# xiezhy6/PASTA-GAN-plusplus

Hardware: AMD Instinct MI355X
Metric: 512-res try-on images/sec (SynthesisNetwork fwd) (higher is better)
Workload: dtype f32

## Files before the change

### include/pasta_gan_ops.h

```cpp
#ifndef PASTA_GAN_OPS_H
#define PASTA_GAN_OPS_H

#include <stdint.h>

#ifdef __cplusplus
extern "C" {
#endif

#define PG_ABI_VERSION 16

enum pg_dtype { PG_F32 = 0, PG_F16 = 1, PG_BF16 = 2, PG_F64 = 3 };

enum pg_error {
    PG_OK = 0,
    PG_ERR_INVALID_ARG = -1,
    PG_ERR_UNSUPPORTED = -2,
    PG_ERR_TOO_LARGE = -3
};

enum pg_act {
    PG_ACT_LINEAR = 1, PG_ACT_RELU = 2, PG_ACT_LRELU = 3, PG_ACT_TANH = 4, PG_ACT_SIGMOID = 5,
    PG_ACT_ELU = 6, PG_ACT_SELU = 7, PG_ACT_SOFTPLUS = 8, PG_ACT_SWISH = 9
};

int pg_bias_act(const void* x, const void* b, const void* xref, const void* yref, const void* dy, void* y,
                int dtype, int64_t sizeX, int sizeB, int64_t stepB,
                int grad, int act, float alpha, float gain, float clamp, void* stream);
int pg_bias_act_abi_version(void);

int64_t pg_bias_act_grad_bias_workspace(int dtype, int64_t sizeX, int sizeB, int64_t stepB);
int pg_bias_act_grad_bias(const void* dy, const void* yref, void* dx, void* db, void* workspace, int64_t workspace_bytes,
                          int dtype, int64_t sizeX, int sizeB, int64_t stepB,
                          int act, float alpha, float gain, float clamp, void* stream);

int pg_upfirdn2d(const void* x, const float* f, void* y, int dtype,
                 int N, int C, int inH, int inW, const int64_t xstride[4],
                 int fh, int fw, const int64_t fstride[2],
                 int outH, int outW, const int64_t ystride[4],
                 int upx, int upy, int downx, int downy, int padx0, int pady0,
                 int flip, float gain, void* stream);
int pg_upfirdn2d_with_odd_samples(const void* x, const float* f, void* y, float* y_odd, int dtype,
                                  int N, int C, int inH, int inW, const int64_t xstride[4],
// ... 86 lines not shown
    float*       s_norm[PG_MODCONV_PREP_MAX_JOBS];
    void*        s16[PG_MODCONV_PREP_MAX_JOBS];
    int          cout[PG_MODCONV_PREP_MAX_JOBS];
    int          cin[PG_MODCONV_PREP_MAX_JOBS];
    int          flags[PG_MODCONV_PREP_MAX_JOBS];
    int          njobs;
    int          half_dtype;
} pg_modconv_prep_jobs;
int pg_modconv_prep_batched(const pg_modconv_prep_jobs* jobs, int N, void* stream);

int pg_conv2d_up2_forward(const float* x, const float* packed, float* y, int N, int Cin, int H, int W, int Cout,
                          const int64_t ystride[4], const float* in_scale, const float* out_scale, void* stream);
int pg_conv2d_up2_splitk_plan(int N, int Cin, int H, int W, int Cout);
int pg_conv2d_up2_forward_splitk(const float* x, const float* packed, float* y, int N, int Cin, int H, int W, int Cout,
                                 const int64_t ystride[4], const float* in_scale, const float* out_scale, float* workspace, int ksplit, void* stream);

int64_t pg_conv2d_up2x3_packed_size(int Cout, int Cin);
int pg_conv2d_up2x3_pack_weight(const float* packed, void* packed_x3, int Cout, int Cin, void* stream);
int pg_conv2d_up2x3_forward(const float* x, const float* packed, const void* packed_x3, float* y, int N, int Cin, int H, int W, int Cout,
                            const int64_t ystride[4], const float* in_scale, const float* out_scale, float* edge_column, void* stream);

int64_t pg_conv2d_stem7x3_packed_size(int Cout);
int pg_conv2d_stem7x3_pack_weight(const float* w, void* packed, int Cout, float scale, int flip_hw, void* stream);
int pg_conv2d_stem7x3_forward(const float* x, const void* packed, float* y, int N, int H, int W, int Cout, const int64_t ystride[4],
                              const pg_conv2d_fusion* fusion, void* stream);

int pg_conv1x1_small(const float* x, const float* w, const float* styles, const float* bias, const float* skip, float* y,
                     int N, int Cin, int64_t HW, int Cout, float scale, float clamp, void* stream);

int pg_conv1x1_fold_prep(const float* wm, const float* bm, const float* wh, const float* bh, const float* styles, float* w_out, float* b_out,
                         int N, int Cm, int C, int Cout, void* stream);
int pg_conv1x1_fold_heads(const float* x, const float* x2, const float* w, const float* bias, const float* skip, float* y_a, float* y_b,
                          int N, int C1, int C2, int64_t HW, int Cout, int c_a, int n_skip, float clamp, void* stream);

int pg_conv3x3_cin1(const float* x, const float* w, float* y, int N, int H, int W, int Cout, float scale, int act, void* stream);

int pg_instance_norm_stats(const float* x, float* mean, float* rstd, int NC, int64_t HW, float eps, void* stream);
int pg_spade_norm(const float* x, const float* mean, const float* rstd, const float* gamma, const float* beta,
                  float* y, int NC, int64_t HW, void* stream);

#define PG_STATS16_MAX_CHUNKS 256
int pg_instance_norm_stats_cl16(const void* x, float* mean, float* rstd, float* workspace, int dtype, int N, int64_t HW, int C, float eps, void* stream);
int pg_spade_combine_cl16(const void* x, const float* mean, const float* rstd, const void* gamma_beta, void* y, int dtype, int N, int64_t HW, int C,
                          int act, float alpha, float gain, float clamp, void* stream);

int pg_spade_train_forward(const float* x, const float* mean, const float* rstd, const float* gamma, const float* beta, float* y,
                           int N, int C, int64_t HW, int64_t gamma_sample_stride, int64_t beta_sample_stride, void* stream);
int pg_spade_train_backward(const float* dy, const float* x, const float* mean, const float* rstd, const float* gamma, float* sums,
                            float* dx, float* dgamma, float* dbeta, int N, int C, int64_t HW,
                            int64_t gamma_sample_stride, int64_t dgamma_sample_stride, int64_t dbeta_sample_stride, void* stream);

int pg_spade_masked_sums(const float* feat, const float* mask, const float* denorm_mask, float* sums, float* counts,
                         int N, int C, int H, int W, void* stream);
int pg_spade_feat_assemble(const float* feat_upper, const float* feat_lower, const float* mask_upper, const float* mask_lower,
                           const float* denorm_mask_upper, const float* denorm_mask_lower,
                           const float* sums_upper, const float* sums_lower, const float* counts_upper, const float* counts_lower,
                           float* out, int N, int C, int H, int W, void* stream);
int pg_conv2d_abi_version(void);
int pg_conv2d_reserve_cus(int n);

int pg_conv2d_wgrad_plan(int N, int Cin, int OH, int OW, int Cout, int KH, int KW, int stride);
int pg_conv2d_wgrad(const float* x, const float* dy, float* dw, float* workspace,
                    int N, int Cin, int H, int W, int Cout, int KH, int KW, int stride, int pad_y, int pad_x, int OH, int OW,
                    int splits, void* stream);

int pg_conv2d16_wgrad_plan(int N, int Cin, int OH, int OW, int Cout, int KH, int KW, int stride);
// ... 213 lines not shown
```

### pasta-gan-plusplus_amd/torch_utils/custom_ops.py

```python

import concurrent.futures
import ctypes
import fcntl
import glob
import hashlib
import os
import re
import shutil
import subprocess
import sys

verbosity = 'brief'

CSRC_DIR = os.path.normpath(os.path.join(os.path.dirname(os.path.abspath(__file__)), '..', 'csrc'))
INCLUDE_DIR = os.path.normpath(os.path.join(CSRC_DIR, '..', '..', 'include'))
DEV_DIR = os.path.join(CSRC_DIR, 'dev')
OFFLOAD_ARCH = 'gfx950'
HIPCC_FLAGS = ['-O3', '-std=c++17', '-fPIC', '-fvisibility=hidden', f'--offload-arch={OFFLOAD_ARCH}']

PLUGIN_SOURCES = {
    'bias_act_plugin': ['bias_act.hip'],
    'upfirdn2d_plugin': ['upfirdn2d.hip'],
    'patch_routing_plugin': ['patch_routing.hip'],
    'augment_plugin': ['augment.hip'],
    'tryon_plugin': ['tryon.hip'],
    'tryon_front_plugin': ['tryon_front.hip'],
    'train_fetch_plugin': ['train_fetch.hip'],
    'snapshot_grid_plugin': ['snapshot_grid.hip'],
    'conv2d_plugin': ['conv2d.hip', 'conv2d_inst_k3s1.hip', 'conv2d_inst_k1s1.hip', 'conv2d_inst_k2x2.hip', 'conv2d_inst_k2x1.hip',
                      'conv2d_inst_k1x2.hip', 'conv2d_inst_k7s1.hip', 'conv2d_inst_k3s2.hip', 'conv2d_inst_k1s2.hip', 'conv2d_inst_wino.hip', 'conv2d_inst_wino4.hip', 'conv2d_inst_wino4s.hip', 'conv2d_inst_wino4t.hip', 'conv2d_inst_wino4x.hip', 'conv2d_inst_wino4xs.hip', 'conv2d_inst_wino4xt.hip', 'conv2d_inst_wino4b.hip', 'conv2d_inst_wino4bs.hip', 'conv2d_inst_up2.hip', 'conv2d_inst_stem7.hip', 'conv2d_inst_s1x1.hip',
                      'conv2d_wgrad.hip', 'conv2d16.hip', 'conv2d16_inst_k3s1.hip', 'conv2d16_inst_k3s1b.hip', 'conv2d16_inst_k1s1.hip', 'conv2d16_inst_k2x2.hip', 'conv2d16_inst_k2x1.hip',
                      'conv2d16_inst_k1x2.hip', 'conv2d16_inst_k3s2.hip', 'conv2d16_inst_up2f.hip', 'conv1x1_head16.hip', 'spade16.hip', 'conv1x1_fold.hip', 'optim.hip'],
}

ABI_VERSION = 16

_cached_plugins = dict()


class NativePlugin:

    def __init__(self, name, path, abi_name=None):
        self.name = name
        self.path = path
        self.lib = ctypes.CDLL(path)
        probe = getattr(self.lib, 'pg_' + (abi_name or name).replace('_plugin', '') + '_abi_version', None)
        if probe is None:
            raise RuntimeError(f'{path} does not export its ABI version; rebuild it from csrc/')
        probe.restype = ctypes.c_int
        if probe() != ABI_VERSION:
            raise RuntimeError(f'{path} implements ABI version {probe()}, the bindings expect {ABI_VERSION}; rebuild it from csrc/')

    def __repr__(self):
        return f'<NativePlugin {self.name} at {self.path}>'


def _find_hipcc():
    for cand in (os.environ.get('HIPCC'), shutil.which('hipcc'), '/opt/rocm/bin/hipcc'):
        if cand and os.path.isfile(cand):
            return cand
    return None


def _digest(sources, extra_flags):
    h = hashlib.md5()
    deps = sorted(set(list(sources) + glob.glob(os.path.join(CSRC_DIR, '*.h')) + glob.glob(os.path.join(INCLUDE_DIR, '*.h'))))
    for path in deps:
        h.update(os.path.basename(path).encode())
# ... 180 lines not shown
```

### pasta-gan-plusplus_amd/torch_utils/ops/conv2d_mfma.py

```python

import ctypes
import os

import torch

from .. import custom_ops
from . import _native as nat

ACT_INDEX = {'linear': 1, 'relu': 2, 'lrelu': 3, 'tanh': 4, 'sigmoid': 5, 'elu': 6, 'selu': 7, 'softplus': 8, 'swish': 9}

FUSED_ACTS = ('linear', 'relu', 'lrelu')

SUPPORTED = {(3, 3, 1), (1, 1, 1), (2, 2, 1), (2, 1, 1), (1, 2, 1), (7, 7, 1), (3, 3, 2), (1, 1, 2)}


class Fusion(ctypes.Structure):
    _fields_ = [
        ('in_scale', ctypes.c_void_p), ('in_bias', ctypes.c_void_p), ('in_act', ctypes.c_int), ('in_alpha', ctypes.c_float),
        ('in_gain', ctypes.c_float), ('in_clamp', ctypes.c_float),
        ('out_scale', ctypes.c_void_p), ('noise', ctypes.c_void_p), ('noise_batch_stride', ctypes.c_int64), ('noise_gain', ctypes.c_float),
        ('bias', ctypes.c_void_p), ('act', ctypes.c_int), ('alpha', ctypes.c_float), ('gain', ctypes.c_float), ('clamp', ctypes.c_float),
        ('residual', ctypes.c_void_p),
        ('spade_x', ctypes.c_void_p), ('spade_mean', ctypes.c_void_p), ('spade_rstd', ctypes.c_void_p),
        ('x2', ctypes.c_void_p), ('cin_split', ctypes.c_int),
# ... 90 lines not shown
        lib.pg_conv2d_wgrad.argtypes = [vp, vp, vp, vp] + [i] * 13 + [vp]
        lib.pg_conv2d_up2_forward.restype = i
        lib.pg_conv2d_up2_forward.argtypes = [vp, vp, vp, i, i, i, i, i, ctypes.POINTER(ctypes.c_int64), vp, vp, vp]
        lib.pg_split3_bf16_cl.restype = i
        lib.pg_split3_bf16_cl.argtypes = [vp, vp, i, i, i64, vp]
        lib.pg_conv2d16_wgrad_x3.restype = i
        lib.pg_conv2d16_wgrad_x3.argtypes = [vp, vp, vp, vp] + [i] * 13 + [vp]
        lib.pg_conv2d16_wgrad_plan.restype = i
        lib.pg_conv2d16_wgrad_plan.argtypes = [i] * 8
        lib.pg_conv2d_up2_splitk_plan.restype = i
        lib.pg_conv2d_up2_splitk_plan.argtypes = [i, i, i, i, i]
        lib.pg_conv2d_up2x3_packed_size.restype = i64
        lib.pg_conv2d_up2x3_packed_size.argtypes = [i, i]
        lib.pg_conv2d_up2x3_pack_weight.restype = i
        lib.pg_conv2d_up2x3_pack_weight.argtypes = [vp, vp, i, i, vp]
        lib.pg_conv2d_up2x3_forward.restype = i
        lib.pg_conv2d_up2x3_forward.argtypes = [vp, vp, vp, vp, i, i, i, i, i, ctypes.POINTER(ctypes.c_int64), vp, vp, vp, vp]
        lib.pg_conv2d_up2_forward_splitk.restype = i
        lib.pg_conv2d_up2_forward_splitk.argtypes = [vp, vp, vp, i, i, i, i, i, ctypes.POINTER(ctypes.c_int64), vp, vp, vp, i, vp]
        lib.pg_conv2d_stem7x3_packed_size.restype = i64
        lib.pg_conv2d_stem7x3_packed_size.argtypes = [i]
        lib.pg_conv2d_stem7x3_pack_weight.restype = i
        lib.pg_conv2d_stem7x3_pack_weight.argtypes = [vp, vp, i, ctypes.c_float, i, vp]
        lib.pg_conv2d_stem7x3_forward.restype = i
        lib.pg_conv2d_stem7x3_forward.argtypes = [vp, vp, vp, i, i, i, i, ctypes.POINTER(ctypes.c_int64), ctypes.POINTER(Fusion), vp]
        lib.pg_conv3x3_cin1.restype = i
        lib.pg_conv3x3_cin1.argtypes = [vp, vp, vp, i, i, i, i, f, i, vp]
        lib.pg_conv1x1_small.restype = i
        lib.pg_conv1x1_small.argtypes = [vp] * 6 + [i, i, i64, i, f, f, vp]
        lib.pg_conv1x1_fold_prep.restype = i
        lib.pg_conv1x1_fold_prep.argtypes = [vp] * 7 + [i, i, i, i, vp]
        lib.pg_conv1x1_fold_heads.restype = i
        lib.pg_conv1x1_fold_heads.argtypes = [vp] * 7 + [i, i, i, i64, i, i, i, f, vp]
        _plugin = plugin
    return _plugin


WINO_F2, WINO_F4, WINO_F4B, WINO_F4X3 = 1, 2, 3, 4
WINO_FORMS = {0: ('direct', False, False), WINO_F2: ('winograd', False, False), WINO_F4: ('winograd4', True, False),
              WINO_F4B: ('winograd4', False, True), WINO_F4X3: ('winograd4x3', True, False)}


def _wino_form(winograd):
    if int(winograd) not in WINO_FORMS:
        raise nat.NativeOpError(f'conv2d_mfma: winograd={winograd!r} is not one of the forms {sorted(WINO_FORMS)}')
    return (int(winograd), *WINO_FORMS[int(winograd)])


_WINO4B = os.environ.get('PG_WINO4B', '1')
F4_FORM = WINO_F4 if _WINO4B == '0' else WINO_F4B
F4_WIDE = WINO_F4 if os.environ.get('PG_WINO4_X3', '1') == '0' else WINO_F4X3


def f4_form(hw):
    if _WINO4B == '2':
        return WINO_F4B
    return F4_FORM if int(hw[1]) < 64 else F4_WIDE


def use_winograd(kh, kw, stride, cout, cin=None, x2=None, pad=None, hw=None, xf=False, ep=None):
    if (int(kh), int(kw), int(stride)) != (3, 3, 1) or x2 is not None:
        return 0
    if pad is not None and not 0 <= int(pad[1]) <= 4:
        return 0
    mode = os.environ.get('PG_CONV_ALGO', 'auto')
    if mode == 'direct':
# ... 480 lines not shown
def conv1x1_fold_prep(wm, bm, wh, bh, styles):
    lib = _init().lib
    wm, bm, wh, bh, styles = _f32c(wm, 'wm'), _f32c(bm, 'bm'), _f32c(wh, 'wh'), _f32c(bh, 'bh'), _f32c(styles, 'styles')
    cm, c = wm.shape
    cout, n = int(wh.shape[0]), int(styles.shape[0])
    if tuple(wh.shape) != (cout, cm) or tuple(styles.shape) != (n, cm) or (bm is not None and bm.numel() != cm) or (bh is not None and bh.numel() != cout):
        raise nat.NativeOpError('conv1x1_fold_prep: wm [Cm, C], bm [Cm], wh [Cout, Cm], bh [Cout], styles [N, Cm]')
    w = torch.empty([n, cout, c], dtype=torch.float32, device=wm.device)
    b = torch.empty([n, cout], dtype=torch.float32, device=wm.device)
    with torch.cuda.device(wm.device):
        rc = lib.pg_conv1x1_fold_prep(nat.ptr(wm), nat.ptr(bm), nat.ptr(wh), nat.ptr(bh), nat.ptr(styles), nat.ptr(w), nat.ptr(b), n, cm, c, cout, nat.stream_of(wm))
    nat.check(rc, 'pg_conv1x1_fold_prep')
    return w, b


def conv1x1_fold_heads(x, x2, w, b, c_a, skip=None, clamp=None):
    lib = _init().lib
    x, x2, w, b, skip = _f32c(x, 'x'), _f32c(x2, 'x2'), _f32c(w, 'w'), _f32c(b, 'b'), _f32c(skip, 'skip')
    n, c1, h, wd = x.shape
    c2, cout, c_a = int(x2.shape[1]), int(w.shape[1]), int(c_a)
    n_skip = int(skip.shape[1]) if skip is not None else 0
    if (tuple(x2.shape) != (n, c2, h, wd) or tuple(w.shape) != (n, cout, c1 + c2) or tuple(b.shape) != (n, cout) or not 0 < c_a <= cout
            or (skip is not None and (tuple(skip.shape) != (n, n_skip, h, wd) or n_skip > cout))):
        raise nat.NativeOpError('conv1x1_fold_heads: x [N, C1, H, W], x2 [N, C2, H, W], w [N, Cout, C1 + C2], b [N, Cout], skip [N, <= Cout, H, W]')
    ya = torch.empty([n, c_a, h, wd], dtype=torch.float32, device=x.device)
    yb = torch.empty([n, cout - c_a, h, wd], dtype=torch.float32, device=x.device) if c_a < cout else None
    with torch.cuda.device(x.device):
        rc = lib.pg_conv1x1_fold_heads(nat.ptr(x), nat.ptr(x2), nat.ptr(w), nat.ptr(b), nat.ptr(skip), nat.ptr(ya), nat.ptr(yb), n, c1, c2, h * wd, cout, c_a,
                                       n_skip, float(clamp) if clamp is not None else -1.0, nat.stream_of(x))
    nat.check(rc, 'pg_conv1x1_fold_heads')
    return ya, yb


def modconv_dcoefs(weight, styles, scale=1.0):
    lib = _init().lib
    weight, styles = _f32c(weight.detach(), 'weight'), _f32c(styles.detach(), 'styles')
    cout, cin, kh, kw = weight.shape
    n = styles.shape[0]
    assert styles.shape[1] == cin
    d = torch.empty([n, cout], dtype=torch.float32, device=weight.device)
    with torch.cuda.device(weight.device):
        st = lib.pg_modconv_dcoefs(nat.ptr(weight), nat.ptr(styles), nat.ptr(d), n, cout, cin, kh * kw, float(scale), nat.stream_of(weight))
    nat.check(st, 'pg_modconv_dcoefs')
    return d


def modconv_w2(weight, scale=1.0):
    lib = _init().lib
    weight = _f32c(weight.detach(), 'weight')
    cout, cin, kh, kw = weight.shape
    w2 = torch.empty([cout, cin], dtype=torch.float32, device=weight.device)
    with torch.cuda.device(weight.device):
        st = lib.pg_modconv_w2(nat.ptr(weight), nat.ptr(w2), cout, cin, kh * kw, float(scale), nat.stream_of(weight))
    nat.check(st, 'pg_modconv_w2')
    return w2


PREP_MAX_JOBS = 32


class PrepJobs(ctypes.Structure):
    _fields_ = [('w2', ctypes.c_void_p * PREP_MAX_JOBS), ('styles', ctypes.c_void_p * PREP_MAX_JOBS), ('out', ctypes.c_void_p * PREP_MAX_JOBS),
                ('s_norm', ctypes.c_void_p * PREP_MAX_JOBS), ('s16', ctypes.c_void_p * PREP_MAX_JOBS), ('cout', ctypes.c_int * PREP_MAX_JOBS),
                ('cin', ctypes.c_int * PREP_MAX_JOBS), ('flags', ctypes.c_int * PREP_MAX_JOBS), ('njobs', ctypes.c_int), ('half_dtype', ctypes.c_int)]


# ... 140 lines not shown
```

### pasta-gan-plusplus_amd/training/networks.py

```python

import os
from typing import NamedTuple, Optional
import numpy as np
import torch
import torch.nn as nn

from torch_utils import misc
from torch_utils.ops import _native as nat
from torch_utils.ops import bias_act
from torch_utils.ops import conv2d_gradfix
from torch_utils.ops import conv2d_mfma
from torch_utils.ops import conv2d_mfma16
from torch_utils.ops import conv2d_resample
from torch_utils.ops import fma
from torch_utils.ops import upfirdn2d

SQRT_HALF = float(np.sqrt(0.5))


def _needs_graph(*tensors):
    return torch.is_grad_enabled() and any(t is not None and t.requires_grad for t in tensors)


def _fast_ok(x, *others):
# ... 850 lines not shown
        beta = self.conv_beta(actv, no_act=True)
        return normalized * (1 + gamma) + beta


    def _forward16(self, x, denorm_feats, post, stats):
        mean, rstd = stats if stats is not None else conv2d_mfma16.instance_norm_stats16(x, eps=self.param_free_norm.eps)
        m, g, b = self.conv_mlp, self.conv_gamma, self.conv_beta
        if (denorm_feats.dtype == torch.float32 and conv2d_mfma.conv3x3_cin1_ok(denorm_feats, m.weight, m.padding) and m.up == 1 and m.down == 1
                and os.environ.get('PG_CIN1_STENCIL', '1') != '0'):
            actv = conv2d_mfma.conv3x3_cin1(denorm_feats, m.weight, scale=m.weight_gain, act='relu').to(dtype=x.dtype, memory_format=torch.channels_last)
        else:
            actv = m(denorm_feats.to(dtype=x.dtype, memory_format=torch.channels_last), no_act=True, post_act='relu')
        c = int(g.weight.shape[0])
        packed = self._cache.get(('gamma_beta16', x.dtype), [g.weight, b.weight],
                                 lambda: conv2d_mfma16.pack_weight(torch.cat([g.weight.detach() * g.weight_gain, b.weight.detach() * b.weight_gain]), x.dtype)[0])
        gb = conv2d_mfma16.conv2d_forward(actv, packed, 2 * c, 3, 3, pad=(g.padding, g.padding))
        return conv2d_mfma16.spade_combine16(x, mean, rstd, gb, **post)


class Spade_ResBlockV4_512(nn.Module):
    def __init__(self, in_channels, out_channels, spade_channels, kernel_size=3, bias=True, activation='linear', up=1, down=1,
                 resample_filter=[1, 3, 3, 1], conv_clamp=None, channels_last=False, trainable=True, resolution=256):
        super().__init__()
        self.register_buffer('resample_filter', upfirdn2d.setup_filter(resample_filter))
        kw = dict(bias=False, resample_filter=resample_filter, conv_clamp=conv_clamp, channels_last=channels_last)
        self.conv = Spade_Conv2dLayer(in_channels, in_channels, kernel_size=3, **kw)
        self.conv0 = Spade_Conv2dLayer(in_channels, out_channels, kernel_size=3, **kw)
        self.conv1 = Spade_Conv2dLayer(out_channels, out_channels, kernel_size=3, **kw)
        self.skip = Spade_Conv2dLayer(in_channels, out_channels, kernel_size=1, **kw)
        self.spade_skip = Spade_Norm_Block(spade_channels, in_channels)
        self.spade0 = Spade_Norm_Block(spade_channels, in_channels)
        self.spade1 = Spade_Norm_Block(spade_channels, out_channels)

    def forward(self, x, denorm_feat):
        if (_fast_ok(x, denorm_feat, self.conv.weight, self.conv0.weight) or _fast16_ok(x, denorm_feat, self.conv.weight, self.conv0.weight)) and all(l.bias is None and l.activation in conv2d_mfma.FUSED_ACTS for l in (self.skip, self.conv0, self.conv1)):
            assert self.spade_skip.param_free_norm.eps == self.spade0.param_free_norm.eps
            x, stats = self.conv(x, no_act=True, stats_eps=self.spade0.param_free_norm.eps)
            y = self.skip(self.spade_skip(x, denorm_feat, post=self.skip.pre_activation(SQRT_HALF), stats=stats), no_act=True)
            x, stats1 = self.conv0(self.spade0(x, denorm_feat, post=self.conv0.pre_activation(), stats=stats), no_act=True, stats_eps=self.spade1.param_free_norm.eps)
            return self.conv1(self.spade1(x, denorm_feat, post=self.conv1.pre_activation(SQRT_HALF), stats=stats1), no_act=True, residual=y)
        x = self.conv(x, no_act=True)
        y = self.skip(self.spade_skip(x, denorm_feat), gain=SQRT_HALF)
        x = self.conv0(self.spade0(x, denorm_feat))
        return self.conv1(self.spade1(x, denorm_feat), gain=SQRT_HALF, residual=y)


class SynthesisLayer(nn.Module):

    def __init__(self, in_channels, out_channels, w_dim, resolution, kernel_size=3, up=1, use_noise=True, activation='lrelu',
                 resample_filter=[1, 3, 3, 1], conv_clamp=None, channels_last=False):
        super().__init__()
        self.resolution, self.up, self.use_noise, self.activation, self.conv_clamp = resolution, up, use_noise, activation, conv_clamp
        self.register_buffer('resample_filter', upfirdn2d.setup_filter(resample_filter))
        self.padding = kernel_size // 2
        self.act_gain = bias_act.activation_funcs[activation].def_gain
        self.affine = FullyConnectedLayer(w_dim, in_channels, bias_init=1)
        memory_format = torch.channels_last if channels_last else torch.contiguous_format
        self.weight = nn.Parameter(torch.randn([out_channels, in_channels, kernel_size, kernel_size]).to(memory_format=memory_format))
        if use_noise:
            self.register_buffer('noise_const', torch.randn([resolution, resolution]))
            self.noise_strength = nn.Parameter(torch.zeros([]))
        self.bias = nn.Parameter(torch.zeros([out_channels]))
        self._cache = _PackCache()

    def forward(self, x, w, noise_mode='random', fused_modconv=True, gain=1, styles=None):
        assert noise_mode in ['random', 'const', 'none']
        in_res = self.resolution // self.up
        misc.assert_shape(x, [None, self.weight.shape[1], in_res, in_res])
        if styles is None:
            styles = self.affine(w)
        noise = None
        if self.use_noise and noise_mode == 'random':
            noise = torch.randn([x.shape[0], 1, self.resolution, self.resolution], device=x.device) * self.noise_strength
        if self.use_noise and noise_mode == 'const':
            if torch.is_grad_enabled() and self.noise_strength.requires_grad:
                noise = self.noise_const * self.noise_strength
            else:
# ... 143 lines not shown
        if (mc.conv_clamp is not None or mc.activation != 'linear' or mc.up != 1 or mc.down != 1 or tuple(mc.weight.shape[2:]) != (1, 1)
                or tuple(tr.weight.shape[2:]) != (1, 1) or int(mc.weight.shape[1]) != int(x.shape[1]) + int(feat.shape[1])):
            return None
        parsing = tr.is_last and tr.is_style
        params = [mc.weight, tr.weight, tr.bias] + ([mc.bias] if mc.bias is not None else []) + ([tr.m_weight1, tr.m_bias1] if parsing else [])
        if not (_fast_ok(x, feat, styles, img, tr.affine.weight, tr.affine.bias, *params) and conv2d_mfma.conv1x1_fold_ok(x, feat, img)):
            return None

        def build():
            cm = int(mc.weight.shape[0])
            heads = [(tr.weight, tr.bias)] + ([(tr.m_weight1, tr.m_bias1)] if parsing else [])
            return ((mc.weight.detach().float().reshape(cm, -1) * mc.weight_gain * mc.act_gain).contiguous(),
                    (mc.bias.detach().float() * mc.act_gain).contiguous() if mc.bias is not None else None,
                    torch.cat([hw.detach().float().reshape(hw.shape[0], cm) for hw, _ in heads]).contiguous(),
                    torch.cat([hb.detach().float() for _, hb in heads]).contiguous())
        wm, bm, wh, bh = self._fold_cache.get(('fold',), params, build)
        if styles is None:
            styles = tr.affine(w) * tr.weight_gain
        try:
            wn, bn = conv2d_mfma.conv1x1_fold_prep(wm, bm, wh, bh, styles)
            return conv2d_mfma.conv1x1_fold_heads(x, feat, wn, bn, int(tr.weight.shape[0]), skip=img, clamp=tr.conv_clamp)
        except nat.NativeNotCovered:
            return None

    def _merge_heads(self, x, feat, w, styles, img, fused_modconv, feat_unused=False):
        if feat_unused:
            heads = self._heads_folded(x, feat, w, styles, img)
            if heads is not None:
                return (None,) + tuple(heads)
        x = self.merge_conv(x, x2=feat)
        rgb, pred_parsing = self.torgb(x, w, fused_modconv=fused_modconv, skip_img=img, styles=styles)
        return x, rgb, pred_parsing

    def _forward(self, x, img, ws, pose_feature, cat_feat, parsing, force_fp32, fused_modconv, styles=None, _feat_unused=False, **layer_kwargs):
        misc.assert_shape(ws, [None, self.num_conv + self.num_torgb, self.w_dim])
        half = (self.use_fp16 or self.half_dtype is not None) and not force_fp32
        fmt = dict(dtype=(self.half_dtype or torch.float16) if half else torch.float32,
                   memory_format=torch.channels_last if ((self.channels_last or self.half_dtype is not None) and not force_fp32) else torch.contiguous_format)
        if fused_modconv is None:
            fused_modconv = (not self.training) and (not half or int(ws.shape[0]) == 1)
        style = lambda i: ws[:, i]
        st = styles if styles is not None else [None] * (self.num_conv + self.num_torgb)
        conv = lambda layer, t, i, **kw: layer(t, style(i), fused_modconv=fused_modconv, styles=st[i], **kw, **layer_kwargs)

        if self.in_channels == 0:
            x = conv(self.conv1, pose_feature.to(**fmt), 0)
        else:
            misc.assert_shape(x, [None, self.in_channels, self.resolution // 2, self.resolution // 2])
            x = x.to(**fmt)
            if self.architecture == 'resnet':
                shortcut = self.skip(x, gain=SQRT_HALF)
                x = conv(self.conv1, conv(self.conv0, x, 0), 1, gain=SQRT_HALF)
                x = shortcut.add_(x)
            else:
                x = conv(self.conv1, conv(self.conv0, x, 0), 1)
                if self.resolution > 32:
                    feat = cat_feat[str(self.resolution)].to(**fmt)
                    if _feat_unused and self.has_torgb and not self.TEXTURE and not half:
                        if img is not None:
                            misc.assert_shape(img, [None, self.img_channels, self.resolution // 2, self.resolution // 2])
                            img = upfirdn2d.upsample2d(img, self.resample_filter)
                        x, rgb, pred_parsing = self._merge_heads(x, feat, style(self.num_conv), st[self.num_conv], img, fused_modconv, feat_unused=True)
                        return x, rgb.to(dtype=torch.float32, memory_format=torch.contiguous_format), pred_parsing
                    x = self.merge_conv(x, x2=feat)
                if self.TEXTURE:
                    x = self.spade_b512(x, parsing)

        if img is not None:
            misc.assert_shape(img, [None, self.img_channels, self.resolution // 2, self.resolution // 2])
            img = upfirdn2d.upsample2d(img, self.resample_filter)
        pred_parsing = None
        if self.has_torgb:
            rgb, pred_parsing = self.torgb(x, style(self.num_conv), fused_modconv=fused_modconv, skip_img=img, styles=st[self.num_conv])
            img = rgb.to(dtype=torch.float32, memory_format=torch.contiguous_format)
        return x, img, pred_parsing


class SynthesisBlockFull_v1_v6(_SynthesisBlockBase):
    TORGB = ToRGBLayerFull_v1_v5

    def forward(self, x, img, ws, pose_feature, cat_feat, force_fp32=False, fused_modconv=None, styles=None, _feat_unused=False, **layer_kwargs):
        return self._forward(x, img, ws, pose_feature, cat_feat, None, force_fp32, fused_modconv, styles=styles, _feat_unused=_feat_unused, **layer_kwargs)


class SynthesisBlockFull_v1_v4(_SynthesisBlockBase):
    TORGB = ToRGBLayerFull_v1_v4
    TEXTURE = True

    def forward(self, x, img, ws, pose_feature, cat_feat, parsing, force_fp32=False, fused_modconv=None, styles=None, **layer_kwargs):
        return self._forward(x, img, ws, pose_feature, cat_feat, parsing, force_fp32, fused_modconv, styles=styles, **layer_kwargs)


def _half_nearest(t):
    return t[:, :, ::2, ::2]


def _batched_affine(owner, entries, ws, num_ws, w_dim):
    n = ws.shape[0]
    params = [t for _, m, _, _ in entries for t in (m.affine.weight, m.affine.bias)]

    def build():
        wt = torch.cat([m.affine.weight.detach().float() * (m.affine.weight_gain * g) for _, m, _, g in entries]).t().contiguous()
        b = torch.cat([m.affine.bias.detach().float() * (m.affine.bias_gain * g) for _, m, _, g in entries]).contiguous()
        return wt, b
    if not hasattr(owner, '_affine_cache'):
        owner._affine_cache, owner._gather = _PackCache(), {}
    wt, b = owner._affine_cache.get(('all',), params, build)
    total = wt.shape[1]
    key = (n, ws.device)
    if key not in owner._gather:
        idx, col = [], 0
        rows = torch.arange(n, dtype=torch.int64)[:, None] * num_ws
        for _, m, wi, _ in entries:
            c = m.affine.weight.shape[0]
            idx.append(((rows + wi) * total + col + torch.arange(c, dtype=torch.int64)[None, :]).reshape(-1))
            col += c
        owner._gather[key] = torch.cat(idx).to(ws.device)
    flat = torch.addmm(b, ws.reshape(n * num_ws, w_dim), wt).reshape(-1).index_select(0, owner._gather[key])
    out, off = {}, 0
    for k, m, _, _ in entries:
        c = m.affine.weight.shape[0]
        out.setdefault(k, []).append(flat[off:off + n * c].view(n, c))
        off += n * c
# ... 93 lines not shown
        finally:
            if pre is not None:
                conv2d_mfma.modconv_prep_clear()

    def _forward_body(self, ws, styles, pre, pose_feat, cat_feat, denorm_upper_input, denorm_lower_input, denorm_upper_mask, denorm_lower_mask, gt_parsing, block_kwargs):
        x = img = pred_parsing = None
        kept = {}
        for res, w in zip(self.block_resolutions, styles):
            block = getattr(self, f'b{res}')
            x, img, pred_parsing = block(x, img, w, pose_feat, cat_feat, force_fp32=not self._half_on(block, ws), styles=pre[res] if pre is not None else None,
                                         _feat_unused=(res == self.block_resolutions[-1]), **block_kwargs)
            kept[res] = (x, img)
        x_256, img_256 = kept[self.block_resolutions[-2]]

        if gt_parsing is not None:
            parsing_index = gt_parsing
        else:
            parsing_index = pred_parsing.detach().argmax(dim=1, keepdim=True).float()
        upper_mask = ((parsing_index == 1) | (parsing_index == 4)).float()
        lower_mask = ((parsing_index == 2) | (parsing_index == 3)).float()

        if _fast_ok(x_256, denorm_upper_input, denorm_lower_input, denorm_upper_mask, denorm_lower_mask) and denorm_upper_mask.dtype == torch.float32:
            feat_u = self.spade_encoder(torch.where(upper_mask > 0.9, denorm_upper_input, -1.0))
            feat_l = self.spade_encoder(torch.where(lower_mask > 0.9, denorm_lower_input, -1.0))
            spade_feat = conv2d_mfma.spade_feat_assemble(feat_u, feat_l, upper_mask, lower_mask, denorm_upper_mask, denorm_lower_mask)
        else:
            spade_feat = (self.get_spade_feat(upper_mask.detach(), denorm_upper_mask, denorm_upper_input) * (_half_nearest(upper_mask) > 0.9)
                          + self.get_spade_feat(lower_mask.detach(), denorm_lower_mask, denorm_lower_input) * (_half_nearest(lower_mask) > 0.9))

        if x_256.dtype != torch.float32:
            spade_feat = spade_feat.to(dtype=x_256.dtype, memory_format=torch.channels_last)
        x_spade = self.spade_b256_2(self.spade_b256_1(x_256, spade_feat), spade_feat)
        _, finetune_img, _ = self.texture_b512(x_spade, img_256, styles[-1], pose_feat, cat_feat, parsing_index, force_fp32=not self._half_on(self.texture_b512, ws),
                                               styles=pre['texture'] if pre is not None else None, **block_kwargs)
        return img, finetune_img, pred_parsing


class SynthesisStackBlock(nn.Module):

    def __init__(self, in_channels, out_channels, w_dim, resolution, img_channels, resample_filter=[1, 3, 3, 1], conv_clamp=None,
                 half_dtype=None, **layer_kwargs):
        super().__init__()
        self.in_channels, self.w_dim, self.resolution, self.img_channels, self.half_dtype = in_channels, w_dim, resolution, img_channels, half_dtype
        self.register_buffer('resample_filter', upfirdn2d.setup_filter(resample_filter))
        layer = dict(w_dim=w_dim, resolution=resolution, conv_clamp=conv_clamp, **layer_kwargs)
        if in_channels == 0:
            self.const = nn.Parameter(torch.randn([out_channels, resolution, resolution]))
        else:
            self.conv0 = SynthesisLayer(in_channels, out_channels, up=2, resample_filter=resample_filter, **layer)
        self.conv1 = SynthesisLayer(out_channels, out_channels, **layer)
        self.torgb = ToRGBLayerFull_v1_v5(out_channels, img_channels, w_dim=w_dim, conv_clamp=conv_clamp)
        self.num_conv = 1 if in_channels == 0 else 2
        self.num_torgb = 1

    def affine_layers(self):
        convs = [self.conv1] if self.in_channels == 0 else [self.conv0, self.conv1]
        return [(m, i, 1.0) for i, m in enumerate(convs)] + [(self.torgb, self.num_conv, self.torgb.weight_gain)]

    def forward(self, x, img, ws, force_fp32=False, styles=None, **layer_kwargs):
        misc.assert_shape(ws, [None, self.num_conv + self.num_torgb, self.w_dim])
        half = self.half_dtype is not None and not force_fp32
        fmt = dict(dtype=self.half_dtype if half else torch.float32, memory_format=torch.channels_last if half else torch.contiguous_format)
        st = list(styles) if styles is not None else [None] * (self.num_conv + self.num_torgb)
        if self.in_channels == 0:
            x = self.const.to(fmt['dtype'])[None].expand(ws.shape[0], -1, -1, -1).contiguous(memory_format=fmt['memory_format'])
            x = self.conv1(x, ws[:, 0], styles=st[0], **layer_kwargs)
        else:
# ... 331 lines not shown
```

Baseline: 278.7.

## Fold texture block tail conv3x3, skip 1x1 and toRGB into one kernel

When the final texture block's feature output is unused, the SPADE residual block defers its last 3x3 conv and 1x1 skip conv. These are algebraically folded with the style-modulated 1x1 toRGB into a single per-sample 3x3+1x1 head with few output channels, computed by a new HIP kernel. This avoids materializing the full-channel 512-res intermediate feature maps and the separate conv launches. The cost is an fp32 CUDA-core kernel with per-sample weights, a clamp applied only after the fold rather than at each stage, and a cached, prepared weight fold.

```diff
diff --git a/include/pasta_gan_ops.h b/include/pasta_gan_ops.h
--- a/include/pasta_gan_ops.h
+++ b/include/pasta_gan_ops.h
@@ -7,7 +7,7 @@
 extern "C" {
 #endif
 
-#define PG_ABI_VERSION 16
+#define PG_ABI_VERSION 17
 
 enum pg_dtype { PG_F32 = 0, PG_F16 = 1, PG_BF16 = 2, PG_F64 = 3 };
 
@@ -160,6 +160,9 @@
                          int N, int Cm, int C, int Cout, void* stream);
 int pg_conv1x1_fold_heads(const float* x, const float* x2, const float* w, const float* bias, const float* skip, float* y_a, float* y_b,
                           int N, int C1, int C2, int64_t HW, int Cout, int c_a, int n_skip, float clamp, void* stream);
+
+int pg_conv3x3_fold_head(const float* xa, const float* xb, const float* w, const float* bias, const float* skip, float* y,
+                         int N, int C, int H, int W, int Cout, float clamp, void* stream);
 
 int pg_conv3x3_cin1(const float* x, const float* w, float* y, int N, int H, int W, int Cout, float scale, int act, void* stream);
 
diff --git a/pasta-gan-plusplus_amd/csrc/conv3x3_fold.hip b/pasta-gan-plusplus_amd/csrc/conv3x3_fold.hip
--- /dev/null
+++ b/pasta-gan-plusplus_amd/csrc/conv3x3_fold.hip
@@ -0,0 +1,151 @@
+#include "pg_common.h"
+
+namespace {
+typedef float f32x4s __attribute__((ext_vector_type(4)));
+typedef unsigned u32x4s __attribute__((ext_vector_type(4)));
+
+constexpr int F3_ROWS = 4;
+constexpr int F3_WAVES = 4;
+constexpr int F3_COLS = 256;
+constexpr int F3_OOB = 0x40000000;
+constexpr int DPP_WAVE_SHL1 = 0x130, DPP_WAVE_SHR1 = 0x138;
+
+template <int CTRL> __device__ __forceinline__ float dpp_or(float old, float v) {
+    return __builtin_bit_cast(float, __builtin_amdgcn_update_dpp(__builtin_bit_cast(int, old), __builtin_bit_cast(int, v), CTRL, 0xf, 0xf, false));
+}
+
+struct F3Planes {
+    f32x4s a[F3_ROWS + 2];
+    float e[F3_ROWS + 2];
+    f32x4s b[F3_ROWS];
+};
+
+template <int CO>
+__global__ __launch_bounds__(256, 2) void conv3x3_fold_head_kernel(const float* __restrict__ xa, const float* __restrict__ xb, const float* __restrict__ w,
+                                                                   const float* __restrict__ bias, const float* __restrict__ skip, float* __restrict__ y,
+                                                                   int C, int H, int W, float clamp) {
+    const int n = blockIdx.z;
+    const int wave = __builtin_amdgcn_readfirstlane((int)threadIdx.x >> 6), lane = (int)threadIdx.x & 63;
+    const int r0 = ((int)blockIdx.y * F3_WAVES + wave) * F3_ROWS;
+    if (r0 >= H) return;
+    const int col = (int)blockIdx.x * F3_COLS + lane * 4;
+    const bool colok = col < W;
+    const int plane_bytes = H * W * 4;
+    const int off_col = colok ? col * 4 : F3_OOB;
+    const int off_edge = lane == 0 ? (col > 0 && colok ? (col - 1) * 4 : F3_OOB) : (lane == 63 && col + 4 < W ? (col + 4) * 4 : F3_OOB);
+    int off_a[F3_ROWS + 2], off_e[F3_ROWS + 2];
+#pragma unroll
+    for (int j = 0; j < F3_ROWS + 2; j++) {
+        const int r = r0 - 1 + j;
+        const int ro = r >= 0 && r < H ? r * W * 4 : F3_OOB;
+        off_a[j] = ro + off_col;
+        off_e[j] = ro + off_edge;
+    }
+    const float* pa = xa + (int64_t)n * C * H * W;
+    const float* pb = xb + (int64_t)n * C * H * W;
+    const float* wn = w + (int64_t)n * CO * 10 * C;
+    const int64_t HW = (int64_t)H * W;
+
+    auto load = [&](int c, F3Planes& p) __attribute__((always_inline)) {
+        const __amdgpu_buffer_rsrc_t ra = __builtin_amdgcn_make_buffer_rsrc(const_cast<float*>(pa + c * HW), 0, plane_bytes, 0x00020000);
+        const __amdgpu_buffer_rsrc_t rb = __builtin_amdgcn_make_buffer_rsrc(const_cast<float*>(pb + c * HW), 0, plane_bytes, 0x00020000);
+#pragma unroll
+        for (int j = 0; j < F3_ROWS + 2; j++) p.a[j] = __builtin_bit_cast(f32x4s, __builtin_amdgcn_raw_buffer_load_b128(ra, off_a[j], 0, 0));
+#pragma unroll
+        for (int j = 0; j < F3_ROWS; j++) p.b[j] = __builtin_bit_cast(f32x4s, __builtin_amdgcn_raw_buffer_load_b128(rb, off_a[j + 1], 0, 0));
+#pragma unroll
+        for (int j = 0; j < F3_ROWS + 2; j++) p.e[j] = __builtin_bit_cast(float, __builtin_amdgcn_raw_buffer_load_b32(ra, off_e[j], 0, 0));
+    };
+
+    float acc[CO][F3_ROWS][4];
+#pragma unroll
+    for (int o = 0; o < CO; o++)
+#pragma unroll
+        for (int t = 0; t < F3_ROWS; t++)
+#pragma unroll
+            for (int q = 0; q < 4; q++) acc[o][t][q] = 0.f;
+
+    auto mac = [&](int c, const F3Planes& p) __attribute__((always_inline)) {
+        float w3[CO][9], w1[CO];
+#pragma unroll
+        for (int o = 0; o < CO; o++) {
+#pragma unroll
+            for (int k = 0; k < 9; k++) w3[o][k] = wn[o * 10 * C + c * 9 + k];
+            w1[o] = wn[o * 10 * C + 9 * C + c];
+        }
+        float v[F3_ROWS + 2][6];
+#pragma unroll
+        for (int j = 0; j < F3_ROWS + 2; j++) {
+            v[j][0] = dpp_or<DPP_WAVE_SHR1>(p.e[j], p.a[j][3]);
+            v[j][1] = p.a[j][0]; v[j][2] = p.a[j][1]; v[j][3] = p.a[j][2]; v[j][4] = p.a[j][3];
+            v[j][5] = dpp_or<DPP_WAVE_SHL1>(p.e[j], p.a[j][0]);
+        }
+#pragma unroll
+        for (int t = 0; t < F3_ROWS; t++) {
+            float part[CO][4];
+#pragma unroll
+            for (int o = 0; o < CO; o++)
+#pragma unroll
+                for (int q = 0; q < 4; q++) part[o][q] = p.b[t][q] * w1[o];
+#pragma unroll
+            for (int ky = 0; ky < 3; ky++)
+#pragma unroll
+                for (int kx = 0; kx < 3; kx++)
+#pragma unroll
+                    for (int o = 0; o < CO; o++)
+#pragma unroll
+                        for (int q = 0; q < 4; q++) part[o][q] = __builtin_fmaf(v[t + ky][q + kx], w3[o][3 * ky + kx], part[o][q]);
+#pragma unroll
+            for (int o = 0; o < CO; o++)
+#pragma unroll
+                for (int q = 0; q < 4; q++) acc[o][t][q] += part[o][q];
+        }
+    };
+
+    F3Planes pA, pB;
+    load(0, pA);
+    int c = 0;
+    for (; c + 1 < C; c += 2) {
+        load(c + 1, pB);
+        __builtin_amdgcn_sched_barrier(0);
+        mac(c, pA);
+        if (c + 2 < C) load(c + 2, pA);
+        __builtin_amdgcn_sched_barrier(0);
+        mac(c + 1, pB);
+    }
+    if (c < C) mac(c, pA);
+
+    if (!colok) return;
+    const float cl = clamp >= 0.f ? clamp : __builtin_inff();
+#pragma unroll
+    for (int o = 0; o < CO; o++) {
+        const float bo = bias[n * CO + o];
+#pragma unroll
+        for (int t = 0; t < F3_ROWS; t++) {
+            if (r0 + t < H) {
+                const int64_t at = (((int64_t)n * CO + o) * H + (r0 + t)) * W + col;
+                f32x4s r;
+#pragma unroll
+                for (int q = 0; q < 4; q++) r[q] = fminf(fmaxf(acc[o][t][q] + bo, -cl), cl);
+                if (skip) r += *(const f32x4s*)(skip + at);
+                *(f32x4s*)(y + at) = r;
+            }
+        }
+    }
+}
+}
+
+PG_EXPORT int pg_conv3x3_fold_head(const float* xa, const float* xb, const float* w, const float* bias, const float* skip, float* y,
+                                   int N, int C, int H, int W, int Cout, float clamp, void* stream) {
+    if (!xa || !xb || !w || !bias || !y || N <= 0 || C <= 0 || H <= 0 || W <= 0 || Cout <= 0) return PG_ERR_INVALID_ARG;
+    if (Cout > 4 || W % 4 != 0 || !pg::aligned16(xa) || !pg::aligned16(xb) || !pg::aligned16(y) || (skip && !pg::aligned16(skip))) return PG_ERR_UNSUPPORTED;
+    if ((int64_t)H * W * 4 > (int64_t)1 << 29 || (int64_t)C * 10 * Cout > (int64_t)1 << 24) return PG_ERR_UNSUPPORTED;
+    const int64_t by = ((int64_t)H + F3_WAVES * F3_ROWS - 1) / (F3_WAVES * F3_ROWS);
+    if (N > 65535 || by > 65535) return PG_ERR_TOO_LARGE;
+    const dim3 grid((unsigned)((W + F3_COLS - 1) / F3_COLS), (unsigned)by, (unsigned)N);
+    hipStream_t s = (hipStream_t)stream;
+#define PG_FOLD3(P) case P: hipLaunchKernelGGL((conv3x3_fold_head_kernel<P>), grid, dim3(64 * F3_WAVES), 0, s, xa, xb, w, bias, skip, y, C, H, W, clamp); break;
+    switch (Cout) { PG_FOLD3(1) PG_FOLD3(2) PG_FOLD3(3) PG_FOLD3(4) }
+#undef PG_FOLD3
+    return pg::launch_status();
+}
diff --git a/pasta-gan-plusplus_amd/torch_utils/custom_ops.py b/pasta-gan-plusplus_amd/torch_utils/custom_ops.py
--- a/pasta-gan-plusplus_amd/torch_utils/custom_ops.py
+++ b/pasta-gan-plusplus_amd/torch_utils/custom_ops.py
@@ -30,10 +30,10 @@
     'conv2d_plugin': ['conv2d.hip', 'conv2d_inst_k3s1.hip', 'conv2d_inst_k1s1.hip', 'conv2d_inst_k2x2.hip', 'conv2d_inst_k2x1.hip',
                       'conv2d_inst_k1x2.hip', 'conv2d_inst_k7s1.hip', 'conv2d_inst_k3s2.hip', 'conv2d_inst_k1s2.hip', 'conv2d_inst_wino.hip', 'conv2d_inst_wino4.hip', 'conv2d_inst_wino4s.hip', 'conv2d_inst_wino4t.hip', 'conv2d_inst_wino4x.hip', 'conv2d_inst_wino4xs.hip', 'conv2d_inst_wino4xt.hip', 'conv2d_inst_wino4b.hip', 'conv2d_inst_wino4bs.hip', 'conv2d_inst_up2.hip', 'conv2d_inst_stem7.hip', 'conv2d_inst_s1x1.hip',
                       'conv2d_wgrad.hip', 'conv2d16.hip', 'conv2d16_inst_k3s1.hip', 'conv2d16_inst_k3s1b.hip', 'conv2d16_inst_k1s1.hip', 'conv2d16_inst_k2x2.hip', 'conv2d16_inst_k2x1.hip',
-                      'conv2d16_inst_k1x2.hip', 'conv2d16_inst_k3s2.hip', 'conv2d16_inst_up2f.hip', 'conv1x1_head16.hip', 'spade16.hip', 'conv1x1_fold.hip', 'optim.hip'],
+                      'conv2d16_inst_k1x2.hip', 'conv2d16_inst_k3s2.hip', 'conv2d16_inst_up2f.hip', 'conv1x1_head16.hip', 'spade16.hip', 'conv1x1_fold.hip', 'conv3x3_fold.hip', 'optim.hip'],
 }
 
-ABI_VERSION = 16
+ABI_VERSION = 17
 
 _cached_plugins = dict()
 
diff --git a/pasta-gan-plusplus_amd/torch_utils/ops/conv2d_mfma.py b/pasta-gan-plusplus_amd/torch_utils/ops/conv2d_mfma.py
--- a/pasta-gan-plusplus_amd/torch_utils/ops/conv2d_mfma.py
+++ b/pasta-gan-plusplus_amd/torch_utils/ops/conv2d_mfma.py
@@ -146,6 +146,8 @@
         lib.pg_conv1x1_fold_prep.argtypes = [vp] * 7 + [i, i, i, i, vp]
         lib.pg_conv1x1_fold_heads.restype = i
         lib.pg_conv1x1_fold_heads.argtypes = [vp] * 7 + [i, i, i, i64, i, i, i, f, vp]
+        lib.pg_conv3x3_fold_head.restype = i
+        lib.pg_conv3x3_fold_head.argtypes = [vp] * 6 + [i, i, i, i, i, f, vp]
         _plugin = plugin
     return _plugin
 
@@ -692,6 +694,28 @@
     return ya, yb
 
 
+def conv3x3_fold_ok(xa, xb, skip=None):
+    return (xa.dtype == torch.float32 and xa.is_cuda and xa.is_contiguous() and xb.dtype == torch.float32 and xb.is_cuda and xb.is_contiguous()
+            and xa.shape == xb.shape
+            and (skip is None or (skip.dtype == torch.float32 and skip.is_cuda and skip.is_contiguous() and skip.shape[0] == xa.shape[0] and skip.shape[2:] == xa.shape[2:])))
+
+
+def conv3x3_fold_head(xa, xb, w, b, skip=None, clamp=None):
+    lib = _init().lib
+    xa, xb, w, b, skip = _f32c(xa, 'xa'), _f32c(xb, 'xb'), _f32c(w, 'w'), _f32c(b, 'b'), _f32c(skip, 'skip')
+    n, c, h, wd = xa.shape
+    cout = int(w.shape[1])
+    if (tuple(xb.shape) != (n, c, h, wd) or tuple(w.shape) != (n, cout, 10 * c) or tuple(b.shape) != (n, cout)
+            or (skip is not None and tuple(skip.shape) != (n, cout, h, wd))):
+        raise nat.NativeOpError('conv3x3_fold_head: xa, xb [N, C, H, W], w [N, Cout, 10 C], b [N, Cout], skip [N, Cout, H, W]')
+    y = torch.empty([n, cout, h, wd], dtype=torch.float32, device=xa.device)
+    with torch.cuda.device(xa.device):
+        rc = lib.pg_conv3x3_fold_head(nat.ptr(xa), nat.ptr(xb), nat.ptr(w), nat.ptr(b), nat.ptr(skip), nat.ptr(y), n, c, h, wd, cout,
+                                      float(clamp) if clamp is not None else -1.0, nat.stream_of(xa))
+    nat.check(rc, 'pg_conv3x3_fold_head')
+    return y
+
+
 def modconv_dcoefs(weight, styles, scale=1.0):
     lib = _init().lib
     weight, styles = _f32c(weight.detach(), 'weight'), _f32c(styles.detach(), 'styles')
diff --git a/pasta-gan-plusplus_amd/training/networks.py b/pasta-gan-plusplus_amd/training/networks.py
--- a/pasta-gan-plusplus_amd/training/networks.py
+++ b/pasta-gan-plusplus_amd/training/networks.py
@@ -906,17 +906,23 @@
         self.spade0 = Spade_Norm_Block(spade_channels, in_channels)
         self.spade1 = Spade_Norm_Block(spade_channels, out_channels)
 
-    def forward(self, x, denorm_feat):
+    def forward(self, x, denorm_feat, _defer_tail=False):
         if (_fast_ok(x, denorm_feat, self.conv.weight, self.conv0.weight) or _fast16_ok(x, denorm_feat, self.conv.weight, self.conv0.weight)) and all(l.bias is None and l.activation in conv2d_mfma.FUSED_ACTS for l in (self.skip, self.conv0, self.conv1)):
             assert self.spade_skip.param_free_norm.eps == self.spade0.param_free_norm.eps
             x, stats = self.conv(x, no_act=True, stats_eps=self.spade0.param_free_norm.eps)
-            y = self.skip(self.spade_skip(x, denorm_feat, post=self.skip.pre_activation(SQRT_HALF), stats=stats), no_act=True)
+            s = self.spade_skip(x, denorm_feat, post=self.skip.pre_activation(SQRT_HALF), stats=stats)
+            defer = _defer_tail and s.dtype == torch.float32
+            y = None if defer else self.skip(s, no_act=True)
             x, stats1 = self.conv0(self.spade0(x, denorm_feat, post=self.conv0.pre_activation(), stats=stats), no_act=True, stats_eps=self.spade1.param_free_norm.eps)
-            return self.conv1(self.spade1(x, denorm_feat, post=self.conv1.pre_activation(SQRT_HALF), stats=stats1), no_act=True, residual=y)
+            h = self.spade1(x, denorm_feat, post=self.conv1.pre_activation(SQRT_HALF), stats=stats1)
+            return (h, s) if defer else self.conv1(h, no_act=True, residual=y)
         x = self.conv(x, no_act=True)
         y = self.skip(self.spade_skip(x, denorm_feat), gain=SQRT_HALF)
         x = self.conv0(self.spade0(x, denorm_feat))
         return self.conv1(self.spade1(x, denorm_feat), gain=SQRT_HALF, residual=y)
+
+    def tail(self, h, s):
+        return self.conv1(h, no_act=True, residual=self.skip(s, no_act=True))
 
 
 class SynthesisLayer(nn.Module):
@@ -1126,6 +1132,46 @@
         rgb, pred_parsing = self.torgb(x, w, fused_modconv=fused_modconv, skip_img=img, styles=styles)
         return x, rgb, pred_parsing
 
+    def _tail_fold_ok(self):
+        sb, tr = getattr(self, 'spade_b512', None), getattr(self, 'torgb', None)
+        if sb is None or tr is None or not self.TEXTURE or torch.is_grad_enabled() or os.environ.get('PG_TEX_FOLD', '1') == '0':
+            return False
+        c1, sk = sb.conv1, sb.skip
+        cm = int(tr.weight.shape[1])
+        return (all(l.bias is None and l.up == 1 and l.down == 1 and int(l.weight.shape[0]) == cm for l in (c1, sk))
+                and tuple(c1.weight.shape[2:]) == (3, 3) and c1.padding == 1 and tuple(sk.weight.shape[2:]) == (1, 1) and sk.padding == 0
+                and c1.weight.shape[1] == sk.weight.shape[1] and tuple(tr.weight.shape[2:]) == (1, 1) and not (tr.is_last and tr.is_style))
+
+    def _tail_folded(self, h, s, w, styles, img):
+        sb, tr = self.spade_b512, self.torgb
+        c1, sk = sb.conv1, sb.skip
+        params = [c1.weight, sk.weight, tr.weight, tr.bias]
+        if not (_fast_ok(h, s, styles, img, tr.affine.weight, tr.affine.bias, *params) and conv2d_mfma.conv3x3_fold_ok(h, s, img)):
+            return None
+
+        def build():
+            cm = int(c1.weight.shape[0])
+            return (torch.cat([(c1.weight.detach().float() * c1.weight_gain).reshape(cm, -1), (sk.weight.detach().float() * sk.weight_gain).reshape(cm, -1)], dim=1).contiguous(),
+                    tr.weight.detach().float().reshape(tr.weight.shape[0], cm).contiguous(), tr.bias.detach().float().contiguous())
+        wm, wh, bh = self._fold_cache.get(('tail',), params, build)
+        if styles is None:
+            styles = tr.affine(w) * tr.weight_gain
+        try:
+            wn, bn = conv2d_mfma.conv1x1_fold_prep(wm, None, wh, bh, styles)
+            return conv2d_mfma.conv3x3_fold_head(h, s, wn, bn, skip=img, clamp=tr.conv_clamp)
+        except nat.NativeNotCovered:
+            return None
+
+    def _spade_heads(self, x, parsing, w, styles, img, fused_modconv, feat_unused=False):
+        x = self.spade_b512(x, parsing, _defer_tail=feat_unused and self._tail_fold_ok())
+        if isinstance(x, tuple):
+            rgb = self._tail_folded(*x, w, styles, img)
+            if rgb is not None:
+                return None, rgb, None
+            x = self.spade_b512.tail(*x)
+        rgb, pred_parsing = self.torgb(x, w, fused_modconv=fused_modconv, skip_img=img, styles=styles)
+        return x, rgb, pred_parsing
+
     def _forward(self, x, img, ws, pose_feature, cat_feat, parsing, force_fp32, fused_modconv, styles=None, _feat_unused=False, **layer_kwargs):
         misc.assert_shape(ws, [None, self.num_conv + self.num_torgb, self.w_dim])
         half = (self.use_fp16 or self.half_dtype is not None) and not force_fp32
@@ -1158,6 +1204,12 @@
                         return x, rgb.to(dtype=torch.float32, memory_format=torch.contiguous_format), pred_parsing
                     x = self.merge_conv(x, x2=feat)
                 if self.TEXTURE:
+                    if _feat_unused and self.has_torgb and not half:
+                        if img is not None:
+                            misc.assert_shape(img, [None, self.img_channels, self.resolution // 2, self.resolution // 2])
+                            img = upfirdn2d.upsample2d(img, self.resample_filter)
+                        x, rgb, pred_parsing = self._spade_heads(x, parsing, style(self.num_conv), st[self.num_conv], img, fused_modconv, feat_unused=True)
+                        return x, rgb.to(dtype=torch.float32, memory_format=torch.contiguous_format), pred_parsing
                     x = self.spade_b512(x, parsing)
 
         if img is not None:
@@ -1181,8 +1233,8 @@
     TORGB = ToRGBLayerFull_v1_v4
     TEXTURE = True
 
-    def forward(self, x, img, ws, pose_feature, cat_feat, parsing, force_fp32=False, fused_modconv=None, styles=None, **layer_kwargs):
-        return self._forward(x, img, ws, pose_feature, cat_feat, parsing, force_fp32, fused_modconv, styles=styles, **layer_kwargs)
+    def forward(self, x, img, ws, pose_feature, cat_feat, parsing, force_fp32=False, fused_modconv=None, styles=None, _feat_unused=False, **layer_kwargs):
+        return self._forward(x, img, ws, pose_feature, cat_feat, parsing, force_fp32, fused_modconv, styles=styles, _feat_unused=_feat_unused, **layer_kwargs)
 
 
 def _half_nearest(t):
@@ -1342,7 +1394,7 @@
             spade_feat = spade_feat.to(dtype=x_256.dtype, memory_format=torch.channels_last)
         x_spade = self.spade_b256_2(self.spade_b256_1(x_256, spade_feat), spade_feat)
         _, finetune_img, _ = self.texture_b512(x_spade, img_256, styles[-1], pose_feat, cat_feat, parsing_index, force_fp32=not self._half_on(self.texture_b512, ws),
-                                               styles=pre['texture'] if pre is not None else None, **block_kwargs)
+                                               styles=pre['texture'] if pre is not None else None, _feat_unused=True, **block_kwargs)
         return img, finetune_img, pred_parsing
 
 
```

Result: faster. 284.9, median of 6 (+2.2%).
